# MDIL-SNU/SevenNet

Hardware: NVIDIA H100
Metric: atom_updates_per_sec (higher is better)
Workload: dtype f32

## Files before the change

sevenn_b200/csrc/engine.cu:

```cuda
#include <algorithm>
#include <cstdlib>
#include <cstring>
#include <functional>
#include <map>
#include <string>
#include <vector>

#include "../../include/sevenn_b200.h"
#include "common.cuh"
#include "conv_kernels.cuh"
#include "edge_kernels.cuh"
#include "neighbor.cuh"
#include "node_kernels.cuh"
#include "tc_gemm.cuh"

namespace s7b {

static thread_local std::string g_error;
static int64_t g_launches = 0;
extern int64_t g_conv_launches;

void set_error(const char* file, int line, const char* msg) {
  char buf[512];
  snprintf(buf, sizeof(buf), "%s:%d: %s", file, line, msg);
// ... 273 lines not shown
static int g_opt_gate_bwd_rows = 0;
static int g_opt_stage_graphs = 0;
static int g_opt_cuda_graph = 1;
static int g_opt_tc_gemm = 1;
static long long* g_tc_trace = nullptr;
static int g_tc_trace_cap = 0;
static int g_opt_tc_swizzle = 1;

__global__ void set_i64_kernel(int64_t* p, int64_t v) { *p = v; }

__global__ void csr_from_sorted_kernel(const int* __restrict__ centre, const int* __restrict__ neighbour,
                                       int64_t n_edges, int n_nodes, int* __restrict__ rowptr,
                                       int* __restrict__ flag) {
  const int64_t e = (int64_t)blockIdx.x * blockDim.x + threadIdx.x;
  if (e > n_edges) return;
  const int prev = (e == 0) ? -1 : centre[e - 1];
  const int cur = (e == n_edges) ? n_nodes : centre[e];
  if (e < n_edges) {
    if (cur < prev || cur < 0 || cur >= n_nodes) { atomicOr(flag, 1); return; }
    const int nb = neighbour[e];
    if (nb < 0 || nb >= n_nodes) atomicOr(flag, 2);
  }
  for (int c = max(prev, -1) + 1; c <= min(cur, n_nodes); ++c) rowptr[c] = (int)e;
}

__global__ void transpose_kernel(const float* __restrict__ in, float* __restrict__ out, int K, int N) {
  const size_t total = (size_t)K * N;
  for (size_t i = (size_t)blockIdx.x * blockDim.x + threadIdx.x; i < total; i += (size_t)gridDim.x * blockDim.x) {
    const int n = (int)(i / K), k = (int)(i - (size_t)n * K);
    out[i] = in[(size_t)k * N + n];
  }
}

struct TcWeights {
  DevBuf q, fb;
  int nblocks = 0;
  bool ok = false;
  struct Blk { int K, N, NT; size_t q_off, fb_off; } blk[kMaxL];
};

static int tc_pick_nt(int N) {
  if (N <= 0) return 0;
  const int tiles = (N + kTcMaxNT - 1) / kTcMaxNT;
  const int w = (N + tiles - 1) / tiles;
  return (w + 15) / 16 * 16;
}
static int tc_tiles(int N, int NT) { return (N + NT - 1) / NT; }

static inline uint16_t bf16_bits_exact(float v) {
  uint32_t u;
  memcpy(&u, &v, 4);
  return (uint16_t)(u >> 16);
}

static void tc_pack_block(const float* W, int K, int N, int NT, uint16_t* q, float* fb) {
  const int n_kc = K / kTcKC;
  for (int n = 0; n < N; ++n) {
    double amax = 0.0;
    for (int k = 0; k < K; ++k) amax = std::max(amax, (double)fabsf(W[(size_t)k * N + n]));
    int Eb = 0;
    const bool zero = !(amax > 1e-30);
    if (!zero) frexp(amax, &Eb);
    fb[n] = zero ? 0.0f : (float)ldexp(1.0, Eb - 7);
    const int nt = n / NT, r = n % NT;
    for (int k = 0; k < K; ++k) {
      double sl[3] = {0.0, 0.0, 0.0};
      if (!zero) {
        const double t = ldexp((double)W[(size_t)k * N + n], 23 - Eb);
        const double q0 = nearbyint(t / 65536.0);
        const double r1 = t - q0 * 65536.0;
        const double q1 = nearbyint(r1 / 256.0);
        const double r2 = r1 - q1 * 256.0;
        const double q2 = nearbyint(r2);
        sl[0] = q0; sl[1] = q1 / 256.0; sl[2] = q2 / 65536.0;
      }
      const int kc = k / kTcKC, kk = k % kTcKC;
      const size_t elem = (size_t)((r & 7) * 16 + (r >> 3) * 512 + (kk >> 3) * 128 + (kk & 7) * 2) / 2;
      for (int sidx = 0; sidx < 3; ++sidx)
        q[(((size_t)nt * n_kc + kc) * 3 + sidx) * ((size_t)NT * kTcKC) + elem] = bf16_bits_exact((float)sl[sidx]);
    }
  }
}

static int tc_build_weights(TcWeights& w, const float* host, const int* Ks, const int* Ns, int n_l) {
  w.ok = false;
  w.nblocks = 0;
  size_t q_total = 0, fb_total = 0, woff = 0;
  for (int l = 0; l < n_l; ++l) {
    const int K = Ks[l], N = Ns[l];
    if (K == 0 || N == 0) continue;
    const int NT = tc_pick_nt(N);
    if (NT == 0 || K % kTcKC != 0) return 0;
    TcWeights::Blk& b = w.blk[w.nblocks++];
    b = {K, N, NT, q_total, fb_total};
    q_total += (size_t)3 * K * NT * tc_tiles(N, NT);
    fb_total += (size_t)N;
  }
  std::vector<uint16_t> q(q_total);
  std::vector<float> fb(fb_total);
  int bi = 0;
  for (int l = 0; l < n_l; ++l) {
    const int K = Ks[l], N = Ns[l];
    if (K == 0 || N == 0) continue;
    const TcWeights::Blk& b = w.blk[bi++];
    tc_pack_block(host + woff, K, N, b.NT, q.data() + b.q_off, fb.data() + b.fb_off);
    woff += (size_t)K * N;
  }
  if (w.q.ensure(q_total * sizeof(uint16_t) + 16) || w.fb.ensure(fb_total * sizeof(float) + 16)) return fail("cudaMalloc failed for tensor-core weights");
  S7B_CUDA_CHECK(cudaMemcpy(w.q.p, q.data(), q_total * sizeof(uint16_t), cudaMemcpyHostToDevice));
  S7B_CUDA_CHECK(cudaMemcpy(w.fb.p, fb.data(), fb_total * sizeof(float), cudaMemcpyHostToDevice));
  w.ok = true;
  return 0;
}

typedef CUresult (*EncodeTiledFn)(CUtensorMap*, CUtensorMapDataType, cuuint32_t, void*, const cuuint64_t*, const cuuint64_t*,
                                  const cuuint32_t*, const cuuint32_t*, CUtensorMapInterleave, CUtensorMapSwizzle,
                                  CUtensorMapL2promotion, CUtensorMapFloatOOBfill);
static EncodeTiledFn tensor_map_encoder() {
  static EncodeTiledFn fn = nullptr;
  if (!fn) {
    void* p = nullptr;
    cudaDriverEntryPointQueryResult q;
    if (cudaGetDriverEntryPoint("cuTensorMapEncodeTiled", &p, cudaEnableDefault, &q) == cudaSuccess && q == cudaDriverEntryPointSuccess)
      fn = reinterpret_cast<EncodeTiledFn>(p);
    else cudaGetLastError();
  }
  return fn;
}

static int launch_row_exponents(RowExp& re, const float* A, int lda, const int* a_off, const int* a_K, int n_l,
                                int n_nodes, cudaStream_t st) {
  RowExpArgs r;
  memset(&r, 0, sizeof(r));
  r.A = A;
  r.lda = lda;
  r.n_nodes = n_nodes;
  int rows = 0;
  for (int l = 0; l < n_l; ++l) {
    if (a_K[l] == 0) continue;
    if (a_K[l] % 4 != 0) return fail("row exponents need K % 4 == 0");
    const int b = r.nblocks++;
    r.d[b] = 2 * l + 1;
    r.K[b] = a_K[l];
    r.a_off[b] = a_off[l];
    r.row_base[b] = rows;
    rows += 2 * l + 1;
  }
  r.rows_per_node = rows;
  re.rows_per_node = rows;
  re.bits = false;
  if (rows == 0 || n_nodes == 0) return 0;
  if (re.buf.ensure((size_t)n_nodes * rows * sizeof(int))) return fail("cudaMalloc failed for row exponents");
  r.E = re.buf.as<int>();
  if (rows > 16) return fail("row exponents: more than 16 rows per node");
  const int blk = 256, wpb = blk / 32;
  row_exponent_kernel<<<(n_nodes + wpb - 1) / wpb, blk, 0, st>>>(r);
  S7B_LAUNCH_CHECK();
  return 0;
}

static int launch_tc_linear(const TcWeights& w, const RowExp& re, const float* A, int lda, const int* a_off,
                            const int* a_K, float* C, int ldc, const int* c_off, const int* c_N, int n_l,
                            int n_nodes, bool accumulate, cudaStream_t st) {
  EncodeTiledFn enc = tensor_map_encoder();
  if (!enc) return fail("cuTensorMapEncodeTiled is unavailable (driver too old?)");
  if (ldc % 4 != 0 || (reinterpret_cast<uintptr_t>(C) & 15) != 0) return fail("tensor-core linear: C rows must be 16-byte aligned");
  for (int l = 0; l < n_l; ++l)
    if (c_N[l] != 0 && a_K[l] != 0 && (c_N[l] % 4 != 0 || c_off[l] % 4 != 0)) return fail("tensor-core linear: output blocks must be multiples of 4 floats");
  TcLinArgs t;
  TcMaps maps;
  memset(&t, 0, sizeof(t));
  memset(&maps, 0, sizeof(maps));
  t.C = C;
  t.E = re.buf.as<int>();
  t.ldc = ldc;
  t.n_nodes = n_nodes;
  t.rows_per_node = re.rows_per_node;
  t.accumulate = accumulate ? 1 : 0;
  t.swizzle = g_opt_tc_swizzle;
  t.e_bits = re.bits ? 1 : 0;
  t.trace = g_tc_trace;
  t.trace_cap = g_tc_trace_cap;
  const int n_mt = (n_nodes + kTcBM - 1) / kTcBM;
  int tiles = 0, rows = 0, bi = 0;
  for (int l = 0; l < n_l; ++l) {
    if (a_K[l] == 0 || c_N[l] == 0) { if (a_K[l] != 0) rows += 2 * l + 1; continue; }
    if (bi >= w.nblocks || w.blk[bi].K != a_K[l] || w.blk[bi].N != c_N[l]) return fail("tensor-core weights do not match the call");
    TcLinBlock& b = t.blk[t.nblocks];
// ... 1339 lines not shown
```

sevenn_b200/csrc/tc_gemm.cuh:

```cuda
#pragma once
#include <cuda.h>
#include <cuda_bf16.h>

#include <type_traits>

#include "common.cuh"
#include "node_kernels.cuh"

namespace s7b {

constexpr int kTcBM = 64;
constexpr int kTcKC = 32;
constexpr int kTcMaxNT = 128;
constexpr int kTcAccRegs = kTcMaxNT / 2;
constexpr int kTcThreads = 320;
constexpr int kTcXformThreads = 128;
constexpr int kTcMmaWarps = 4;
constexpr int kTcRawBytes = kTcBM * kTcKC * 4;
constexpr int kTcASliceBytes = kTcBM * kTcKC * 2;
constexpr int kTcBSliceBytes = kTcMaxNT * kTcKC * 2;
constexpr int kTcRawStages = 4, kTcOpsStages = 3, kTcWStages = 5;
constexpr int kTcOpsBytes = 3 * kTcASliceBytes, kTcWBytes = 3 * kTcBSliceBytes;
constexpr int kTcCBox = 16;
constexpr int kTcCBoxBytes = kTcBM * kTcCBox * 4;
constexpr int kTcCBytes = kTcBM * kTcMaxNT * 4;
constexpr int kTcRawOff = 0;
constexpr int kTcOpsOff = kTcRawOff + kTcRawStages * kTcRawBytes;
constexpr int kTcWOff = kTcOpsOff + kTcOpsStages * kTcOpsBytes;
constexpr int kTcCOff = kTcWOff + kTcWStages * kTcWBytes;
constexpr int kTcSmemBytes = kTcCOff + kTcCBytes + 1024 ;
static_assert(kTcCOff % 1024 == 0, "the swizzled C staging tile must be 1024-byte aligned");
constexpr int kTcZeroRow = -1000;

__device__ __forceinline__ uint32_t smem_u32(const void* p) {
  return static_cast<uint32_t>(__cvta_generic_to_shared(p));
}
__device__ __forceinline__ void mbar_init(uint64_t* bar, uint32_t count) {
  asm volatile("mbarrier.init.shared::cta.b64 [%0], %1;" ::"r"(smem_u32(bar)), "r"(count) : "memory");
}
__device__ __forceinline__ void mbar_wait(uint64_t* bar, uint32_t parity) {
  asm volatile(
      "{\n"
      ".reg .pred P1;\n"
      "LAB_WAIT:\n"
      "mbarrier.try_wait.parity.shared::cta.b64 P1, [%0], %1;\n"
      "@P1 bra DONE;\n"
      "bra LAB_WAIT;\n"
      "DONE:\n"
      "}\n" ::"r"(smem_u32(bar)), "r"(parity) : "memory");
}
__device__ __forceinline__ void mbar_arrive(uint64_t* bar) {
  asm volatile("mbarrier.arrive.shared::cta.b64 _, [%0];" ::"r"(smem_u32(bar)) : "memory");
}
__device__ __forceinline__ void mbar_arrive_after(uint64_t* bar, float dep) {
  asm volatile(
      "{\n"
      ".reg .pred p;\n"
      "setp.ne.b32 p, %1, 0x7fc12345;\n"
      "@p mbarrier.arrive.shared::cta.b64 _, [%0];\n"
      "}\n" ::"r"(smem_u32(bar)), "r"(__float_as_uint(dep)) : "memory");
}
__device__ __forceinline__ void mbar_expect_tx(uint64_t* bar, uint32_t bytes) {
  asm volatile("mbarrier.arrive.expect_tx.shared::cta.b64 _, [%0], %1;" ::"r"(smem_u32(bar)), "r"(bytes) : "memory");
}
__device__ __forceinline__ void fence_async_smem() { asm volatile("fence.proxy.async.shared::cta;" ::: "memory"); }

__device__ __forceinline__ void tma_load_3d(void* dst, const CUtensorMap* map, int c0, int c1, int c2, uint64_t* bar) {
  asm volatile(
      "cp.async.bulk.tensor.3d.shared::cluster.global.tile.mbarrier::complete_tx::bytes [%0], [%1, {%2, %3, %4}], [%5];"
      ::"r"(smem_u32(dst)), "l"(reinterpret_cast<uint64_t>(map)), "r"(c0), "r"(c1), "r"(c2), "r"(smem_u32(bar))
      : "memory");
}
__device__ __forceinline__ void bulk_load(void* dst, const void* src, uint32_t bytes, uint64_t* bar) {
  asm volatile(
      "cp.async.bulk.shared::cluster.global.mbarrier::complete_tx::bytes [%0], [%1], %2, [%3];"
      ::"r"(smem_u32(dst)), "l"(reinterpret_cast<uint64_t>(src)), "r"(bytes), "r"(smem_u32(bar))
      : "memory");
}
__device__ __forceinline__ void tma_store_3d(const CUtensorMap* map, uint32_t src, int c0, int c1, int c2) {
  asm volatile("cp.async.bulk.tensor.3d.global.shared::cta.tile.bulk_group [%0, {%1, %2, %3}], [%4];"
               ::"l"(reinterpret_cast<uint64_t>(map)), "r"(c0), "r"(c1), "r"(c2), "r"(src) : "memory");
}
__device__ __forceinline__ void tma_reduce_add_3d(const CUtensorMap* map, uint32_t src, int c0, int c1, int c2) {
  asm volatile("cp.reduce.async.bulk.tensor.3d.global.shared::cta.add.tile.bulk_group [%0, {%1, %2, %3}], [%4];"
               ::"l"(reinterpret_cast<uint64_t>(map)), "r"(c0), "r"(c1), "r"(c2), "r"(src) : "memory");
}
__device__ __forceinline__ void bulk_commit() { asm volatile("cp.async.bulk.commit_group;" ::: "memory"); }
__device__ __forceinline__ void bulk_wait_read_all() { asm volatile("cp.async.bulk.wait_group.read 0;" ::: "memory"); }
__device__ __forceinline__ void bulk_wait_all() { asm volatile("cp.async.bulk.wait_group 0;" ::: "memory"); }
__device__ __forceinline__ void mma_group_sync() { asm volatile("bar.sync 1, 128;" ::: "memory"); }
__device__ __forceinline__ void sts64(uint32_t saddr, float x, float y) {
  asm volatile("st.shared.v2.f32 [%0], {%1, %2};" ::"r"(saddr), "f"(x), "f"(y) : "memory");
}

__device__ __forceinline__ uint64_t gmma_desc(uint32_t saddr) {
  return (uint64_t)((saddr & 0x3FFFF) >> 4) | ((uint64_t)(128 >> 4) << 16) | ((uint64_t)(512 >> 4) << 32);
}
__device__ __forceinline__ void wgmma_fence() { asm volatile("wgmma.fence.sync.aligned;" ::: "memory"); }
__device__ __forceinline__ void wgmma_commit() { asm volatile("wgmma.commit_group.sync.aligned;" ::: "memory"); }
template <int N>
__device__ __forceinline__ void wgmma_wait() { asm volatile("wgmma.wait_group.sync.aligned %0;" ::"n"(N) : "memory"); }
__device__ __forceinline__ void acc_fence(float (&d)[kTcAccRegs]) {
#pragma unroll
  for (int i = 0; i < kTcAccRegs; ++i) asm volatile("" : "+f"(d[i])::"memory");
}
template <int N>
__device__ __forceinline__ void wgmma_bf16(float (&d)[kTcAccRegs], uint64_t da, uint64_t db, uint32_t scale_d);
template <> __device__ __forceinline__ void wgmma_bf16<16>(float (&d)[kTcAccRegs], uint64_t da, uint64_t db, uint32_t scale_d) {
  asm volatile(
      "{\n.reg .pred p;\nsetp.ne.b32 p, %10, 0;\n"
      "wgmma.mma_async.sync.aligned.m64n16k16.f32.bf16.bf16 {%0, %1, %2, %3, %4, %5, %6, %7}, %8, %9, p, 1, 1, 0, 0;\n}\n"
      : "+f"(d[0]), "+f"(d[1]), "+f"(d[2]), "+f"(d[3]), "+f"(d[4]), "+f"(d[5]), "+f"(d[6]), "+f"(d[7])
      : "l"(da), "l"(db), "r"(scale_d));
}
template <> __device__ __forceinline__ void wgmma_bf16<32>(float (&d)[kTcAccRegs], uint64_t da, uint64_t db, uint32_t scale_d) {
  asm volatile(
      "{\n.reg .pred p;\nsetp.ne.b32 p, %18, 0;\n"
      "wgmma.mma_async.sync.aligned.m64n32k16.f32.bf16.bf16 {%0, %1, %2, %3, %4, %5, %6, %7, %8, %9, %10, %11, %12, %13, %14, %15}, %16, %17, p, 1, 1, 0, 0;\n}\n"
      : "+f"(d[0]), "+f"(d[1]), "+f"(d[2]), "+f"(d[3]), "+f"(d[4]), "+f"(d[5]), "+f"(d[6]), "+f"(d[7]), "+f"(d[8]), "+f"(d[9]), "+f"(d[10]), "+f"(d[11]), "+f"(d[12]), "+f"(d[13]), "+f"(d[14]), "+f"(d[15])
      : "l"(da), "l"(db), "r"(scale_d));
}
template <> __device__ __forceinline__ void wgmma_bf16<48>(float (&d)[kTcAccRegs], uint64_t da, uint64_t db, uint32_t scale_d) {
  asm volatile(
      "{\n.reg .pred p;\nsetp.ne.b32 p, %26, 0;\n"
      "wgmma.mma_async.sync.aligned.m64n48k16.f32.bf16.bf16 {%0, %1, %2, %3, %4, %5, %6, %7, %8, %9, %10, %11, %12, %13, %14, %15, %16, %17, %18, %19, %20, %21, %22, %23}, %24, %25, p, 1, 1, 0, 0;\n}\n"
      : "+f"(d[0]), "+f"(d[1]), "+f"(d[2]), "+f"(d[3]), "+f"(d[4]), "+f"(d[5]), "+f"(d[6]), "+f"(d[7]), "+f"(d[8]), "+f"(d[9]), "+f"(d[10]), "+f"(d[11]), "+f"(d[12]), "+f"(d[13]), "+f"(d[14]), "+f"(d[15]), "+f"(d[16]), "+f"(d[17]), "+f"(d[18]), "+f"(d[19]), "+f"(d[20]), "+f"(d[21]), "+f"(d[22]), "+f"(d[23])
      : "l"(da), "l"(db), "r"(scale_d));
}
template <> __device__ __forceinline__ void wgmma_bf16<64>(float (&d)[kTcAccRegs], uint64_t da, uint64_t db, uint32_t scale_d) {
  asm volatile(
      "{\n.reg .pred p;\nsetp.ne.b32 p, %34, 0;\n"
      "wgmma.mma_async.sync.aligned.m64n64k16.f32.bf16.bf16 {%0, %1, %2, %3, %4, %5, %6, %7, %8, %9, %10, %11, %12, %13, %14, %15, %16, %17, %18, %19, %20, %21, %22, %23, %24, %25, %26, %27, %28, %29, %30, %31}, %32, %33, p, 1, 1, 0, 0;\n}\n"
      : "+f"(d[0]), "+f"(d[1]), "+f"(d[2]), "+f"(d[3]), "+f"(d[4]), "+f"(d[5]), "+f"(d[6]), "+f"(d[7]), "+f"(d[8]), "+f"(d[9]), "+f"(d[10]), "+f"(d[11]), "+f"(d[12]), "+f"(d[13]), "+f"(d[14]), "+f"(d[15]), "+f"(d[16]), "+f"(d[17]), "+f"(d[18]), "+f"(d[19]), "+f"(d[20]), "+f"(d[21]), "+f"(d[22]), "+f"(d[23]), "+f"(d[24]), "+f"(d[25]), "+f"(d[26]), "+f"(d[27]), "+f"(d[28]), "+f"(d[29]), "+f"(d[30]), "+f"(d[31])
      : "l"(da), "l"(db), "r"(scale_d));
}
template <> __device__ __forceinline__ void wgmma_bf16<80>(float (&d)[kTcAccRegs], uint64_t da, uint64_t db, uint32_t scale_d) {
  asm volatile(
      "{\n.reg .pred p;\nsetp.ne.b32 p, %42, 0;\n"
      "wgmma.mma_async.sync.aligned.m64n80k16.f32.bf16.bf16 {%0, %1, %2, %3, %4, %5, %6, %7, %8, %9, %10, %11, %12, %13, %14, %15, %16, %17, %18, %19, %20, %21, %22, %23, %24, %25, %26, %27, %28, %29, %30, %31, %32, %33, %34, %35, %36, %37, %38, %39}, %40, %41, p, 1, 1, 0, 0;\n}\n"
      : "+f"(d[0]), "+f"(d[1]), "+f"(d[2]), "+f"(d[3]), "+f"(d[4]), "+f"(d[5]), "+f"(d[6]), "+f"(d[7]), "+f"(d[8]), "+f"(d[9]), "+f"(d[10]), "+f"(d[11]), "+f"(d[12]), "+f"(d[13]), "+f"(d[14]), "+f"(d[15]), "+f"(d[16]), "+f"(d[17]), "+f"(d[18]), "+f"(d[19]), "+f"(d[20]), "+f"(d[21]), "+f"(d[22]), "+f"(d[23]), "+f"(d[24]), "+f"(d[25]), "+f"(d[26]), "+f"(d[27]), "+f"(d[28]), "+f"(d[29]), "+f"(d[30]), "+f"(d[31]), "+f"(d[32]), "+f"(d[33]), "+f"(d[34]), "+f"(d[35]), "+f"(d[36]), "+f"(d[37]), "+f"(d[38]), "+f"(d[39])
      : "l"(da), "l"(db), "r"(scale_d));
}
template <> __device__ __forceinline__ void wgmma_bf16<96>(float (&d)[kTcAccRegs], uint64_t da, uint64_t db, uint32_t scale_d) {
  asm volatile(
      "{\n.reg .pred p;\nsetp.ne.b32 p, %50, 0;\n"
      "wgmma.mma_async.sync.aligned.m64n96k16.f32.bf16.bf16 {%0, %1, %2, %3, %4, %5, %6, %7, %8, %9, %10, %11, %12, %13, %14, %15, %16, %17, %18, %19, %20, %21, %22, %23, %24, %25, %26, %27, %28, %29, %30, %31, %32, %33, %34, %35, %36, %37, %38, %39, %40, %41, %42, %43, %44, %45, %46, %47}, %48, %49, p, 1, 1, 0, 0;\n}\n"
      : "+f"(d[0]), "+f"(d[1]), "+f"(d[2]), "+f"(d[3]), "+f"(d[4]), "+f"(d[5]), "+f"(d[6]), "+f"(d[7]), "+f"(d[8]), "+f"(d[9]), "+f"(d[10]), "+f"(d[11]), "+f"(d[12]), "+f"(d[13]), "+f"(d[14]), "+f"(d[15]), "+f"(d[16]), "+f"(d[17]), "+f"(d[18]), "+f"(d[19]), "+f"(d[20]), "+f"(d[21]), "+f"(d[22]), "+f"(d[23]), "+f"(d[24]), "+f"(d[25]), "+f"(d[26]), "+f"(d[27]), "+f"(d[28]), "+f"(d[29]), "+f"(d[30]), "+f"(d[31]), "+f"(d[32]), "+f"(d[33]), "+f"(d[34]), "+f"(d[35]), "+f"(d[36]), "+f"(d[37]), "+f"(d[38]), "+f"(d[39]), "+f"(d[40]), "+f"(d[41]), "+f"(d[42]), "+f"(d[43]), "+f"(d[44]), "+f"(d[45]), "+f"(d[46]), "+f"(d[47])
      : "l"(da), "l"(db), "r"(scale_d));
}
template <> __device__ __forceinline__ void wgmma_bf16<112>(float (&d)[kTcAccRegs], uint64_t da, uint64_t db, uint32_t scale_d) {
  asm volatile(
      "{\n.reg .pred p;\nsetp.ne.b32 p, %58, 0;\n"
      "wgmma.mma_async.sync.aligned.m64n112k16.f32.bf16.bf16 {%0, %1, %2, %3, %4, %5, %6, %7, %8, %9, %10, %11, %12, %13, %14, %15, %16, %17, %18, %19, %20, %21, %22, %23, %24, %25, %26, %27, %28, %29, %30, %31, %32, %33, %34, %35, %36, %37, %38, %39, %40, %41, %42, %43, %44, %45, %46, %47, %48, %49, %50, %51, %52, %53, %54, %55}, %56, %57, p, 1, 1, 0, 0;\n}\n"
      : "+f"(d[0]), "+f"(d[1]), "+f"(d[2]), "+f"(d[3]), "+f"(d[4]), "+f"(d[5]), "+f"(d[6]), "+f"(d[7]), "+f"(d[8]), "+f"(d[9]), "+f"(d[10]), "+f"(d[11]), "+f"(d[12]), "+f"(d[13]), "+f"(d[14]), "+f"(d[15]), "+f"(d[16]), "+f"(d[17]), "+f"(d[18]), "+f"(d[19]), "+f"(d[20]), "+f"(d[21]), "+f"(d[22]), "+f"(d[23]), "+f"(d[24]), "+f"(d[25]), "+f"(d[26]), "+f"(d[27]), "+f"(d[28]), "+f"(d[29]), "+f"(d[30]), "+f"(d[31]), "+f"(d[32]), "+f"(d[33]), "+f"(d[34]), "+f"(d[35]), "+f"(d[36]), "+f"(d[37]), "+f"(d[38]), "+f"(d[39]), "+f"(d[40]), "+f"(d[41]), "+f"(d[42]), "+f"(d[43]), "+f"(d[44]), "+f"(d[45]), "+f"(d[46]), "+f"(d[47]), "+f"(d[48]), "+f"(d[49]), "+f"(d[50]), "+f"(d[51]), "+f"(d[52]), "+f"(d[53]), "+f"(d[54]), "+f"(d[55])
      : "l"(da), "l"(db), "r"(scale_d));
}
template <> __device__ __forceinline__ void wgmma_bf16<128>(float (&d)[kTcAccRegs], uint64_t da, uint64_t db, uint32_t scale_d) {
  asm volatile(
      "{\n.reg .pred p;\nsetp.ne.b32 p, %66, 0;\n"
      "wgmma.mma_async.sync.aligned.m64n128k16.f32.bf16.bf16 {%0, %1, %2, %3, %4, %5, %6, %7, %8, %9, %10, %11, %12, %13, %14, %15, %16, %17, %18, %19, %20, %21, %22, %23, %24, %25, %26, %27, %28, %29, %30, %31, %32, %33, %34, %35, %36, %37, %38, %39, %40, %41, %42, %43, %44, %45, %46, %47, %48, %49, %50, %51, %52, %53, %54, %55, %56, %57, %58, %59, %60, %61, %62, %63}, %64, %65, p, 1, 1, 0, 0;\n}\n"
      : "+f"(d[0]), "+f"(d[1]), "+f"(d[2]), "+f"(d[3]), "+f"(d[4]), "+f"(d[5]), "+f"(d[6]), "+f"(d[7]), "+f"(d[8]), "+f"(d[9]), "+f"(d[10]), "+f"(d[11]), "+f"(d[12]), "+f"(d[13]), "+f"(d[14]), "+f"(d[15]), "+f"(d[16]), "+f"(d[17]), "+f"(d[18]), "+f"(d[19]), "+f"(d[20]), "+f"(d[21]), "+f"(d[22]), "+f"(d[23]), "+f"(d[24]), "+f"(d[25]), "+f"(d[26]), "+f"(d[27]), "+f"(d[28]), "+f"(d[29]), "+f"(d[30]), "+f"(d[31]), "+f"(d[32]), "+f"(d[33]), "+f"(d[34]), "+f"(d[35]), "+f"(d[36]), "+f"(d[37]), "+f"(d[38]), "+f"(d[39]), "+f"(d[40]), "+f"(d[41]), "+f"(d[42]), "+f"(d[43]), "+f"(d[44]), "+f"(d[45]), "+f"(d[46]), "+f"(d[47]), "+f"(d[48]), "+f"(d[49]), "+f"(d[50]), "+f"(d[51]), "+f"(d[52]), "+f"(d[53]), "+f"(d[54]), "+f"(d[55]), "+f"(d[56]), "+f"(d[57]), "+f"(d[58]), "+f"(d[59]), "+f"(d[60]), "+f"(d[61]), "+f"(d[62]), "+f"(d[63])
      : "l"(da), "l"(db), "r"(scale_d));
}

__device__ __forceinline__ float exp2i(int e) {
  e = e < -126 ? -126 : (e > 127 ? 127 : e);
  return __int_as_float((e + 127) << 23);
}

struct RowExpArgs {
  const float* A;
  int* E;
  int lda, n_nodes, rows_per_node, nblocks;
  int d[kMaxL], K[kMaxL], a_off[kMaxL], row_base[kMaxL];
};

__global__ void row_exponent_kernel(const RowExpArgs a) {
  __shared__ unsigned int smax[8][16];
  const int wib = threadIdx.x >> 5, lane = threadIdx.x & 31;
  const int n = blockIdx.x * (blockDim.x >> 5) + wib;
  if (lane < 16) smax[wib][lane] = 0u;
  __syncwarp();
  if (n < a.n_nodes) {
    for (int b = 0; b < a.nblocks; ++b) {
      const int K = a.K[b], quads = (a.d[b] * K) >> 2;
      const float4* row = reinterpret_cast<const float4*>(a.A + (size_t)n * a.lda + a.a_off[b]);
      for (int q0 = 0; q0 < quads; q0 += 32) {
        const int q = q0 + lane;
        unsigned int m = 0u;
        int r = -1;
        if (q < quads) {
          const float4 v = __ldg(row + q);
          m = __float_as_uint(v.x) & 0x7fffffffu;
          m = max(m, __float_as_uint(v.y) & 0x7fffffffu);
          m = max(m, __float_as_uint(v.z) & 0x7fffffffu);
          m = max(m, __float_as_uint(v.w) & 0x7fffffffu);
          r = a.row_base[b] + (4 * q) / K;
        }
        const unsigned int peers = __match_any_sync(0xffffffffu, r);
        const unsigned int mm = __reduce_max_sync(peers, m);
        if (r >= 0 && lane == __ffs(peers) - 1) smax[wib][r] = max(smax[wib][r], mm);
        __syncwarp();
      }
    }
  }
  __syncwarp();
  if (n < a.n_nodes && lane < a.rows_per_node) {
    const int ex = (int)(smax[wib][lane] >> 23);
    a.E[(size_t)n * a.rows_per_node + lane] = (ex == 0 || ex == 255) ? kTcZeroRow : max(ex - 126, -104);
  }
}

struct TcLinBlock {
  const uint16_t* Wq;
  const float* fb;
  int d, K, N, NT, nnt;
  int c_off, c_cs;
  int row_base;
  int tile0;
};
struct TcLinArgs {
  float* C;
  const int* E;
  int ldc, n_nodes, rows_per_node, accumulate, nblocks, n_tiles, swizzle;
  int e_bits;
  long long* trace;
  int trace_cap;
  TcLinBlock blk[kMaxL];
};
#define TC_TRACE(role, ev, idx)                                                                   \
  do {                                                                                            \
    if (a.trace != nullptr && blockIdx.x == 0) {                                                  \
      const int per = a.trace_cap / 5;                                                            \
      if (trace_n < per) {                                                                        \
        long long* rec = a.trace + 8 + 3 * ((size_t)(role) * per + trace_n);                      \
        rec[0] = (ev);                                                                            \
        rec[1] = (long long)(idx);                                                                \
        rec[2] = clock64();                                                                       \
        ++trace_n;                                                                                \
        a.trace[1 + (role)] = trace_n;                                                            \
      }                                                                                           \
    }                                                                                             \
  } while (0)
struct TcMaps { CUtensorMap m[kMaxL], c[kMaxL]; };

__device__ __forceinline__ float4 lds128(uint32_t saddr) {
  float4 v;
  asm volatile("ld.shared.v4.f32 {%0, %1, %2, %3}, [%4];" : "=f"(v.x), "=f"(v.y), "=f"(v.z), "=f"(v.w) : "r"(saddr) : "memory");
  return v;
}
__device__ __forceinline__ void sts128(uint32_t saddr, uint32_t a, uint32_t b, uint32_t c, uint32_t d) {
  asm volatile("st.shared.v4.b32 [%0], {%1, %2, %3, %4};" ::"r"(saddr), "r"(a), "r"(b), "r"(c), "r"(d) : "memory");
}

__device__ __forceinline__ uint32_t pack_bf16(float lo, float hi) {
  const __nv_bfloat162 v = __floats2bfloat162_rn(lo, hi);
  return *reinterpret_cast<const uint32_t*>(&v);
}

template <int N>
__device__ __forceinline__ void tc_mma_chunk(float (&acc0)[kTcAccRegs], float (&acc1)[kTcAccRegs], uint32_t sa,
                                             uint32_t sb, bool first) {
  constexpr uint32_t b_slice = (uint32_t)N * kTcKC * 2u;
#pragma unroll
  for (int j = 0; j < kTcKC / 16; ++j) {
    const uint32_t ko = (uint32_t)j * 256u;
    const uint64_t dA0 = gmma_desc(sa + ko);
    const uint64_t dA1 = gmma_desc(sa + kTcASliceBytes + ko);
    const uint64_t dA2 = gmma_desc(sa + 2 * kTcASliceBytes + ko);
    const uint64_t dB0 = gmma_desc(sb + ko);
    const uint64_t dB1 = gmma_desc(sb + b_slice + ko);
    const uint64_t dB2 = gmma_desc(sb + 2 * b_slice + ko);
    const uint32_t acc = (!first || j > 0) ? 1u : 0u;
    wgmma_bf16<N>(acc0, dA0, dB0, acc);
    wgmma_bf16<N>(acc1, dA0, dB1, acc);
    wgmma_bf16<N>(acc1, dA1, dB0, 1u);
    wgmma_bf16<N>(acc1, dA0, dB2, 1u);
    wgmma_bf16<N>(acc1, dA1, dB1, 1u);
    wgmma_bf16<N>(acc1, dA2, dB0, 1u);
  }
}

__global__ void __launch_bounds__(kTcThreads, 1)
blocklin_tc_kernel(const TcLinArgs a, const __grid_constant__ TcMaps maps) {
  extern __shared__ uint8_t smem_raw[];
  uint8_t* smem = reinterpret_cast<uint8_t*>((reinterpret_cast<uintptr_t>(smem_raw) + 1023) & ~(uintptr_t)1023);
  __shared__ uint64_t bar_raw_full[kTcRawStages], bar_raw_empty[kTcRawStages];
  __shared__ uint64_t bar_ops_full[kTcOpsStages], bar_ops_empty[kTcOpsStages];
  __shared__ uint64_t bar_w_full[kTcWStages], bar_w_empty[kTcWStages];
  __shared__ __align__(16) float fb_s[kTcMaxNT];

  const int tid = threadIdx.x, warp = tid >> 5, lane = tid & 31;
  int trace_n = 0;

  if (tid == 0) {
    for (int s = 0; s < kTcRawStages; ++s) { mbar_init(&bar_raw_full[s], 1); mbar_init(&bar_raw_empty[s], kTcXformThreads); }
    for (int s = 0; s < kTcOpsStages; ++s) { mbar_init(&bar_ops_full[s], kTcXformThreads); mbar_init(&bar_ops_empty[s], kTcMmaWarps); }
    for (int s = 0; s < kTcWStages; ++s) { mbar_init(&bar_w_full[s], 1); mbar_init(&bar_w_empty[s], kTcMmaWarps); }
    asm volatile("fence.mbarrier_init.release.cluster;" ::: "memory");
  }
  __syncthreads();

  auto decode = [&](int t, int& b, int& mt, int& ci, int& nt) {
    b = 0;
    while (b + 1 < a.nblocks && t >= a.blk[b + 1].tile0) ++b;
    const int rel = t - a.blk[b].tile0;
    const int nnt = a.blk[b].nnt;
    nt = rel % nnt;
    const int r2 = rel / nnt;
    ci = r2 % a.blk[b].d;
    mt = r2 / a.blk[b].d;
  };
  auto row_exp = [&](int t, int row) -> int {
    if (t >= a.n_tiles) return kTcZeroRow;
    int b, mt, ci, nt;
    decode(t, b, mt, ci, nt);
    const int node = mt * kTcBM + row;
    if (node >= a.n_nodes) return kTcZeroRow;
    int v = __ldg(a.E + (size_t)node * a.rows_per_node + a.blk[b].row_base + ci);
    if (a.e_bits) {
      const int ex = v >> 23;
      v = (ex == 0 || ex == 255) ? kTcZeroRow : max(ex - 126, -104);
    }
    return v;
  };

  if (warp == 8) {
    if (lane == 0) {
      uint32_t it = 0;
      for (int t = blockIdx.x; t < a.n_tiles; t += gridDim.x) {
        int b, mt, ci, nt;
        decode(t, b, mt, ci, nt);
        const int n_kc = a.blk[b].K / kTcKC;
        for (int kc = 0; kc < n_kc; ++kc, ++it) {
          const int s = it % kTcRawStages;
          mbar_wait(&bar_raw_empty[s], ((it / kTcRawStages) & 1) ^ 1);
          TC_TRACE(0, 0, it);
          mbar_expect_tx(&bar_raw_full[s], (uint32_t)kTcRawBytes);
          tma_load_3d(smem + kTcRawOff + (size_t)s * kTcRawBytes, &maps.m[b], kc * kTcKC, ci, mt * kTcBM, &bar_raw_full[s]);
        }
      }
    }
  } else if (warp == 9) {
    if (lane == 0) {
      uint32_t it = 0;
      for (int t = blockIdx.x; t < a.n_tiles; t += gridDim.x) {
        int b, mt, ci, nt;
        decode(t, b, mt, ci, nt);
        const TcLinBlock& B = a.blk[b];
        const int n_kc = B.K / kTcKC;
        const uint32_t b_bytes = 3u * (uint32_t)B.NT * kTcKC * 2u;
        const uint8_t* wsrc = reinterpret_cast<const uint8_t*>(B.Wq) + (size_t)nt * n_kc * b_bytes;
        for (int kc = 0; kc < n_kc; ++kc, ++it) {
          const int s = it % kTcWStages;
          mbar_wait(&bar_w_empty[s], ((it / kTcWStages) & 1) ^ 1);
          TC_TRACE(4, 0, it);
          mbar_expect_tx(&bar_w_full[s], b_bytes);
          bulk_load(smem + kTcWOff + (size_t)s * kTcWBytes, wsrc + (size_t)kc * b_bytes, b_bytes, &bar_w_full[s]);
        }
      }
    }
  } else if (warp < 4) {
    const int r = tid & (kTcBM - 1), h = tid / kTcBM;
    const uint32_t swz = a.swizzle ? (uint32_t)(r & 7) : 0u;
    const uint32_t row_off = (uint32_t)((r & 7) * 16 + (r >> 3) * 512);
    const V2 M2 = splat2(12582912.0f), nM2 = splat2(-12582912.0f);
    uint32_t it = 0;
    int Ea_next = row_exp(blockIdx.x, r);
    for (int t = blockIdx.x; t < a.n_tiles; t += gridDim.x) {
      int b, mt, ci, nt;
      decode(t, b, mt, ci, nt);
      const int n_kc = a.blk[b].K / kTcKC;
      const int Ea = Ea_next;
      Ea_next = row_exp(t + gridDim.x, r);
      const float sc = (Ea == kTcZeroRow) ? 0.0f : exp2i(23 - Ea);
      for (int kc = 0; kc < n_kc; ++kc, ++it) {
        const int s = it % kTcRawStages, o = it % kTcOpsStages;
        mbar_wait(&bar_raw_full[s], (it / kTcRawStages) & 1);
        if (tid == 0) TC_TRACE(1, 0, it);
        const uint32_t raw = smem_u32(smem + kTcRawOff + (size_t)s * kTcRawBytes + (size_t)r * 128);
        float4 v[4];
#pragma unroll
        for (int q = 0; q < 4; ++q) v[q] = lds128(raw + (((uint32_t)(4 * h + q) ^ swz) << 4));
        const float dep = (v[0].x + v[1].x) + (v[2].x + v[3].x);
        mbar_arrive_after(&bar_raw_empty[s], dep);
        mbar_wait(&bar_ops_empty[o], ((it / kTcOpsStages) & 1) ^ 1);
        if (tid == 0) TC_TRACE(1, 1, it);
        const uint32_t a0 = smem_u32(smem + kTcOpsOff + (size_t)o * kTcOpsBytes);
        const uint32_t a1 = a0 + kTcASliceBytes, a2 = a1 + kTcASliceBytes;
#pragma unroll
        for (int kk = 0; kk < 2; ++kk) {
          const V2 x[4] = {make_float2(v[2 * kk].x, v[2 * kk].y), make_float2(v[2 * kk].z, v[2 * kk].w),
                           make_float2(v[2 * kk + 1].x, v[2 * kk + 1].y), make_float2(v[2 * kk + 1].z, v[2 * kk + 1].w)};
          uint32_t p0[4], p1[4], p2[4];
#pragma unroll
          for (int j = 0; j < 4; ++j) {
            const V2 tt = mul_(x[j], sc);
            const V2 q0 = add_(fma_(tt, splat2(1.52587890625e-05f), M2), nM2);
            const V2 r1 = fma_(q0, splat2(-65536.0f), tt);
            const V2 q1 = add_(fma_(r1, splat2(0.00390625f), M2), nM2);
            const V2 r2 = fma_(q1, splat2(-256.0f), r1);
            const V2 q2 = add_(add_(r2, M2), nM2);
            const V2 s1 = mul_(q1, 0.00390625f), s2 = mul_(q2, 1.52587890625e-05f);
            p0[j] = pack_bf16(q0.x, q0.y);
            p1[j] = pack_bf16(s1.x, s1.y);
            p2[j] = pack_bf16(s2.x, s2.y);
          }
          const uint32_t off = row_off + (uint32_t)(2 * h + kk) * 128u;
          sts128(a0 + off, p0[0], p0[1], p0[2], p0[3]);
          sts128(a1 + off, p1[0], p1[1], p1[2], p1[3]);
          sts128(a2 + off, p2[0], p2[1], p2[2], p2[3]);
        }
        fence_async_smem();
        if (tid == 0) TC_TRACE(1, 2, it);
        mbar_arrive(&bar_ops_full[o]);
      }
    }
  } else if (warp < 8) {
    const int mw = warp - 4, q4 = lane & 3, ct = tid - 128;
    const int rl = 16 * mw + (lane >> 2);
    const uint32_t cst = smem_u32(smem + kTcCOff);
    auto c_addr = [&](int r, int j) -> uint32_t {
      const int g = 2 * (j & 1) + (q4 >> 1);
      return cst + (uint32_t)((j >> 1) * kTcCBoxBytes + r * 64 + ((g ^ ((r >> 1) & 3)) << 4) + (q4 & 1) * 8);
    };
    float acc0[kTcAccRegs], acc1[kTcAccRegs];
#pragma unroll
    for (int i = 0; i < kTcAccRegs; ++i) { acc0[i] = 0.0f; acc1[i] = 0.0f; }
    uint32_t it = 0, tile_it = 0;
    int Ea_next0 = row_exp(blockIdx.x, rl), Ea_next1 = row_exp(blockIdx.x, rl + 8);
    for (int t = blockIdx.x; t < a.n_tiles; t += gridDim.x, ++tile_it) {
      int b, mt, ci, nt;
      decode(t, b, mt, ci, nt);
      const TcLinBlock& B = a.blk[b];
      const int n_kc = B.K / kTcKC;
      const int Ea0 = Ea_next0, Ea1 = Ea_next1;
      Ea_next0 = row_exp(t + gridDim.x, rl);
      Ea_next1 = row_exp(t + gridDim.x, rl + 8);
      const int col0 = nt * B.NT;
      const float fb_t = (ct < B.NT && col0 + ct < B.N) ? __ldg(B.fb + col0 + ct) : 0.0f;
      auto run_tile = [&](auto width) {
        constexpr int N = decltype(width)::value;
        int prev_o = 0, prev_w = 0;
        for (int kc = 0; kc < n_kc; ++kc, ++it) {
          const int o = it % kTcOpsStages, w = it % kTcWStages;
          mbar_wait(&bar_w_full[w], (it / kTcWStages) & 1);
          if (tid == 128) TC_TRACE(2, 0, it);
          mbar_wait(&bar_ops_full[o], (it / kTcOpsStages) & 1);
          if (tid == 128) TC_TRACE(2, 1, it);
          __syncwarp();
          const uint32_t sa = smem_u32(smem + kTcOpsOff + (size_t)o * kTcOpsBytes);
          const uint32_t sb = smem_u32(smem + kTcWOff + (size_t)w * kTcWBytes);
          acc_fence(acc0);
          acc_fence(acc1);
          wgmma_fence();
          tc_mma_chunk<N>(acc0, acc1, sa, sb, kc == 0);
          wgmma_commit();
          acc_fence(acc0);
          acc_fence(acc1);
          wgmma_wait<1>();
          if (kc > 0) {
            __syncwarp();
            if (lane == 0) { mbar_arrive(&bar_ops_empty[prev_o]); mbar_arrive(&bar_w_empty[prev_w]); }
          }
          prev_o = o;
          prev_w = w;
        }
        wgmma_wait<0>();
        acc_fence(acc0);
        acc_fence(acc1);
        __syncwarp();
        if (lane == 0) { mbar_arrive(&bar_ops_empty[prev_o]); mbar_arrive(&bar_w_empty[prev_w]); }
        if (tid == 160) TC_TRACE(3, 0, tile_it);

        const float fa0 = (Ea0 == kTcZeroRow) ? 0.0f : exp2i(Ea0 - 7);
        const float fa1 = (Ea1 == kTcZeroRow) ? 0.0f : exp2i(Ea1 - 7);
        if (tid == 128) bulk_wait_read_all();
        fb_s[ct] = fb_t;
        mma_group_sync();
        if (tid == 160) TC_TRACE(3, 2, tile_it);
#pragma unroll
        for (int j = 0; j < N / 8; ++j) {
          const float2 fb2 = *reinterpret_cast<const float2*>(&fb_s[8 * j + 2 * q4]);
          sts64(c_addr(rl, j), (acc0[4 * j + 0] + acc1[4 * j + 0]) * fa0 * fb2.x,
                (acc0[4 * j + 1] + acc1[4 * j + 1]) * fa0 * fb2.y);
          sts64(c_addr(rl + 8, j), (acc0[4 * j + 2] + acc1[4 * j + 2]) * fa1 * fb2.x,
                (acc0[4 * j + 3] + acc1[4 * j + 3]) * fa1 * fb2.y);
        }
        if (tid == 160) TC_TRACE(3, 3, tile_it);
      };
      switch (B.NT) {
        case 16: run_tile(std::integral_constant<int, 16>()); break;
        case 32: run_tile(std::integral_constant<int, 32>()); break;
        case 48: run_tile(std::integral_constant<int, 48>()); break;
        case 64: run_tile(std::integral_constant<int, 64>()); break;
        case 80: run_tile(std::integral_constant<int, 80>()); break;
        case 96: run_tile(std::integral_constant<int, 96>()); break;
        case 112: run_tile(std::integral_constant<int, 112>()); break;
        default: run_tile(std::integral_constant<int, 128>()); break;
      }
      fence_async_smem();
      mma_group_sync();
      if (tid == 128) {
        for (int s = 0; s < B.NT / kTcCBox && col0 + s * kTcCBox < B.N; ++s) {
          const uint32_t src = cst + (uint32_t)(s * kTcCBoxBytes);
          if (a.accumulate) tma_reduce_add_3d(&maps.c[b], src, col0 + s * kTcCBox, ci, mt * kTcBM);
          else tma_store_3d(&maps.c[b], src, col0 + s * kTcCBox, ci, mt * kTcBM);
        }
        bulk_commit();
      }
      if (tid == 160) TC_TRACE(3, 1, tile_it);
    }
    if (tid == 128) bulk_wait_all();
  }
}

}
```

Baseline: 1.414 million.

## Ping-pong two MMA warpgroups with dedicated store warp and 64B swizzled operands

Adds a second consumer warpgroup so two MMA groups alternate tiles, each running its epilogue while the other runs tensor-core MMAs. A dedicated warp now issues the TMA stores and reduce-adds for the C staging tile. setmaxnreg rebalances registers toward the MMA warps. Weights and transformed A operands are also switched to a 64-byte swizzled shared-memory layout to cut bank conflicts. The cost is more threads and more mbarrier coordination. The single C staging buffer is still shared between the groups, so their epilogues serialize on it.

```diff
diff --git a/sevenn_b200/csrc/engine.cu b/sevenn_b200/csrc/engine.cu
--- a/sevenn_b200/csrc/engine.cu
+++ b/sevenn_b200/csrc/engine.cu
@@ -379,6 +379,17 @@
   }
 }
 
+static void tc_swizzle_block(uint16_t* q, size_t elems, int NT) {
+  const size_t piece = (size_t)NT * kTcKC;
+  std::vector<uint16_t> tmp(piece);
+  for (size_t p0 = 0; p0 < elems; p0 += piece) {
+    for (int r = 0; r < NT; ++r)
+      for (int g = 0; g < kTcKC / 8; ++g)
+        memcpy(tmp.data() + tc_swz64((uint32_t)r, (uint32_t)g) / 2, q + p0 + ((r & 7) * 16 + (r >> 3) * 512 + g * 128) / 2, 16);
+    memcpy(q + p0, tmp.data(), piece * sizeof(uint16_t));
+  }
+}
+
 static int tc_build_weights(TcWeights& w, const float* host, const int* Ks, const int* Ns, int n_l) {
   w.ok = false;
   w.nblocks = 0;
@@ -401,6 +412,7 @@
     if (K == 0 || N == 0) continue;
     const TcWeights::Blk& b = w.blk[bi++];
     tc_pack_block(host + woff, K, N, b.NT, q.data() + b.q_off, fb.data() + b.fb_off);
+    tc_swizzle_block(q.data() + b.q_off, (size_t)3 * K * b.NT * tc_tiles(N, b.NT), b.NT);
     woff += (size_t)K * N;
   }
   if (w.q.ensure(q_total * sizeof(uint16_t) + 16) || w.fb.ensure(fb_total * sizeof(float) + 16)) return fail("cudaMalloc failed for tensor-core weights");
diff --git a/sevenn_b200/csrc/tc_gemm.cuh b/sevenn_b200/csrc/tc_gemm.cuh
--- a/sevenn_b200/csrc/tc_gemm.cuh
+++ b/sevenn_b200/csrc/tc_gemm.cuh
@@ -13,7 +13,8 @@
 constexpr int kTcKC = 32;
 constexpr int kTcMaxNT = 128;
 constexpr int kTcAccRegs = kTcMaxNT / 2;
-constexpr int kTcThreads = 320;
+constexpr int kTcThreads = 512;
+constexpr int kTcXformRegs = 88, kTcProdRegs = 40, kTcMmaRegs = 192;
 constexpr int kTcXformThreads = 128;
 constexpr int kTcMmaWarps = 4;
 constexpr int kTcRawBytes = kTcBM * kTcKC * 4;
@@ -88,14 +89,17 @@
 __device__ __forceinline__ void bulk_commit() { asm volatile("cp.async.bulk.commit_group;" ::: "memory"); }
 __device__ __forceinline__ void bulk_wait_read_all() { asm volatile("cp.async.bulk.wait_group.read 0;" ::: "memory"); }
 __device__ __forceinline__ void bulk_wait_all() { asm volatile("cp.async.bulk.wait_group 0;" ::: "memory"); }
-__device__ __forceinline__ void mma_group_sync() { asm volatile("bar.sync 1, 128;" ::: "memory"); }
+__device__ __forceinline__ void mma_group_sync(int g) { asm volatile("bar.sync %0, 128;" ::"r"(1 + g) : "memory"); }
+template <int R> __device__ __forceinline__ void setmaxnreg_inc() { asm volatile("setmaxnreg.inc.sync.aligned.u32 %0;" ::"n"(R)); }
+template <int R> __device__ __forceinline__ void setmaxnreg_dec() { asm volatile("setmaxnreg.dec.sync.aligned.u32 %0;" ::"n"(R)); }
 __device__ __forceinline__ void sts64(uint32_t saddr, float x, float y) {
   asm volatile("st.shared.v2.f32 [%0], {%1, %2};" ::"r"(saddr), "f"(x), "f"(y) : "memory");
 }
 
 __device__ __forceinline__ uint64_t gmma_desc(uint32_t saddr) {
-  return (uint64_t)((saddr & 0x3FFFF) >> 4) | ((uint64_t)(128 >> 4) << 16) | ((uint64_t)(512 >> 4) << 32);
-}
+  return (uint64_t)((saddr & 0x3FFFF) >> 4) | ((uint64_t)1 << 16) | ((uint64_t)(512 >> 4) << 32) | ((uint64_t)2 << 62);
+}
+__host__ __device__ __forceinline__ uint32_t tc_swz64(uint32_t r, uint32_t g) { return r * 64u + ((g ^ ((r >> 1) & 3u)) << 4); }
 __device__ __forceinline__ void wgmma_fence() { asm volatile("wgmma.fence.sync.aligned;" ::: "memory"); }
 __device__ __forceinline__ void wgmma_commit() { asm volatile("wgmma.commit_group.sync.aligned;" ::: "memory"); }
 template <int N>
@@ -231,7 +235,7 @@
 #define TC_TRACE(role, ev, idx)                                                                   \
   do {                                                                                            \
     if (a.trace != nullptr && blockIdx.x == 0) {                                                  \
-      const int per = a.trace_cap / 5;                                                            \
+      const int per = a.trace_cap / 7;                                                            \
       if (trace_n < per) {                                                                        \
         long long* rec = a.trace + 8 + 3 * ((size_t)(role) * per + trace_n);                      \
         rec[0] = (ev);                                                                            \
@@ -264,7 +268,7 @@
   constexpr uint32_t b_slice = (uint32_t)N * kTcKC * 2u;
 #pragma unroll
   for (int j = 0; j < kTcKC / 16; ++j) {
-    const uint32_t ko = (uint32_t)j * 256u;
+    const uint32_t ko = (uint32_t)j * 32u;
     const uint64_t dA0 = gmma_desc(sa + ko);
     const uint64_t dA1 = gmma_desc(sa + kTcASliceBytes + ko);
     const uint64_t dA2 = gmma_desc(sa + 2 * kTcASliceBytes + ko);
@@ -288,7 +292,9 @@
   __shared__ uint64_t bar_raw_full[kTcRawStages], bar_raw_empty[kTcRawStages];
   __shared__ uint64_t bar_ops_full[kTcOpsStages], bar_ops_empty[kTcOpsStages];
   __shared__ uint64_t bar_w_full[kTcWStages], bar_w_empty[kTcWStages];
-  __shared__ __align__(16) float fb_s[kTcMaxNT];
+  __shared__ uint64_t bar_c_full, bar_c_free[2];
+  __shared__ uint64_t bar_turn[2];
+  __shared__ __align__(16) float fb_s[2][kTcMaxNT];
 
   const int tid = threadIdx.x, warp = tid >> 5, lane = tid & 31;
   int trace_n = 0;
@@ -297,6 +303,11 @@
     for (int s = 0; s < kTcRawStages; ++s) { mbar_init(&bar_raw_full[s], 1); mbar_init(&bar_raw_empty[s], kTcXformThreads); }
     for (int s = 0; s < kTcOpsStages; ++s) { mbar_init(&bar_ops_full[s], kTcXformThreads); mbar_init(&bar_ops_empty[s], kTcMmaWarps); }
     for (int s = 0; s < kTcWStages; ++s) { mbar_init(&bar_w_full[s], 1); mbar_init(&bar_w_empty[s], kTcMmaWarps); }
+    mbar_init(&bar_c_full, 1);
+    mbar_init(&bar_c_free[0], 1);
+    mbar_init(&bar_c_free[1], 1);
+    mbar_init(&bar_turn[0], kTcMmaWarps);
+    mbar_init(&bar_turn[1], kTcMmaWarps);
     asm volatile("fence.mbarrier_init.release.cluster;" ::: "memory");
   }
   __syncthreads();
@@ -325,8 +336,9 @@
     return v;
   };
 
-  if (warp == 8) {
-    if (lane == 0) {
+  if (warp >= 4 && warp < 8) {
+    setmaxnreg_dec<kTcProdRegs>();
+    if (warp == 4 && lane == 0) {
       uint32_t it = 0;
       for (int t = blockIdx.x; t < a.n_tiles; t += gridDim.x) {
         int b, mt, ci, nt;
@@ -340,9 +352,7 @@
           tma_load_3d(smem + kTcRawOff + (size_t)s * kTcRawBytes, &maps.m[b], kc * kTcKC, ci, mt * kTcBM, &bar_raw_full[s]);
         }
       }
-    }
-  } else if (warp == 9) {
-    if (lane == 0) {
+    } else if (warp == 5 && lane == 0) {
       uint32_t it = 0;
       for (int t = blockIdx.x; t < a.n_tiles; t += gridDim.x) {
         int b, mt, ci, nt;
@@ -359,11 +369,30 @@
           bulk_load(smem + kTcWOff + (size_t)s * kTcWBytes, wsrc + (size_t)kc * b_bytes, b_bytes, &bar_w_full[s]);
         }
       }
+    } else if (warp == 6 && lane == 0) {
+      uint32_t s = 0;
+      for (int t = blockIdx.x; t < a.n_tiles; t += gridDim.x, ++s) {
+        int b, mt, ci, nt;
+        decode(t, b, mt, ci, nt);
+        const TcLinBlock& B = a.blk[b];
+        const int col0 = nt * B.NT;
+        mbar_wait(&bar_c_full, s & 1);
+        const uint32_t cst = smem_u32(smem + kTcCOff);
+        for (int q = 0; q < B.NT / kTcCBox && col0 + q * kTcCBox < B.N; ++q) {
+          const uint32_t src = cst + (uint32_t)(q * kTcCBoxBytes);
+          if (a.accumulate) tma_reduce_add_3d(&maps.c[b], src, col0 + q * kTcCBox, ci, mt * kTcBM);
+          else tma_store_3d(&maps.c[b], src, col0 + q * kTcCBox, ci, mt * kTcBM);
+        }
+        bulk_commit();
+        bulk_wait_read_all();
+        mbar_arrive(&bar_c_free[(s + 1) & 1]);
+      }
+      bulk_wait_all();
     }
   } else if (warp < 4) {
+    setmaxnreg_dec<kTcXformRegs>();
     const int r = tid & (kTcBM - 1), h = tid / kTcBM;
     const uint32_t swz = a.swizzle ? (uint32_t)(r & 7) : 0u;
-    const uint32_t row_off = (uint32_t)((r & 7) * 16 + (r >> 3) * 512);
     const V2 M2 = splat2(12582912.0f), nM2 = splat2(-12582912.0f);
     uint32_t it = 0;
     int Ea_next = row_exp(blockIdx.x, r);
@@ -406,7 +435,7 @@
             p1[j] = pack_bf16(s1.x, s1.y);
             p2[j] = pack_bf16(s2.x, s2.y);
           }
-          const uint32_t off = row_off + (uint32_t)(2 * h + kk) * 128u;
+          const uint32_t off = tc_swz64((uint32_t)r, (uint32_t)(2 * h + kk));
           sts128(a0 + off, p0[0], p0[1], p0[2], p0[3]);
           sts128(a1 + off, p1[0], p1[1], p1[2], p1[3]);
           sts128(a2 + off, p2[0], p2[1], p2[2], p2[3]);
@@ -416,27 +445,29 @@
         mbar_arrive(&bar_ops_full[o]);
       }
     }
-  } else if (warp < 8) {
-    const int mw = warp - 4, q4 = lane & 3, ct = tid - 128;
+  } else {
+    setmaxnreg_inc<kTcMmaRegs>();
+    const int g = (warp - 8) >> 2, mw = (warp - 8) & 3, q4 = lane & 3, ct = tid & 127;
     const int rl = 16 * mw + (lane >> 2);
+    const bool tr_mma = (ct == 0), tr_epi = (ct == 32);
+    const int role_mma = g ? 5 : 2, role_epi = g ? 6 : 3;
     const uint32_t cst = smem_u32(smem + kTcCOff);
+    float* fbs = fb_s[g];
     auto c_addr = [&](int r, int j) -> uint32_t {
-      const int g = 2 * (j & 1) + (q4 >> 1);
-      return cst + (uint32_t)((j >> 1) * kTcCBoxBytes + r * 64 + ((g ^ ((r >> 1) & 3)) << 4) + (q4 & 1) * 8);
+      const int gr = 2 * (j & 1) + (q4 >> 1);
+      return cst + (uint32_t)((j >> 1) * kTcCBoxBytes + r * 64 + ((gr ^ ((r >> 1) & 3)) << 4) + (q4 & 1) * 8);
     };
     float acc0[kTcAccRegs], acc1[kTcAccRegs];
 #pragma unroll
     for (int i = 0; i < kTcAccRegs; ++i) { acc0[i] = 0.0f; acc1[i] = 0.0f; }
-    uint32_t it = 0, tile_it = 0;
-    int Ea_next0 = row_exp(blockIdx.x, rl), Ea_next1 = row_exp(blockIdx.x, rl + 8);
+    uint32_t it = 0, tile_it = 0, mine = 0;
     for (int t = blockIdx.x; t < a.n_tiles; t += gridDim.x, ++tile_it) {
       int b, mt, ci, nt;
       decode(t, b, mt, ci, nt);
       const TcLinBlock& B = a.blk[b];
       const int n_kc = B.K / kTcKC;
-      const int Ea0 = Ea_next0, Ea1 = Ea_next1;
-      Ea_next0 = row_exp(t + gridDim.x, rl);
-      Ea_next1 = row_exp(t + gridDim.x, rl + 8);
+      if ((int)(tile_it & 1) != g) { it += n_kc; continue; }
+      const int Ea0 = row_exp(t, rl), Ea1 = row_exp(t, rl + 8);
       const int col0 = nt * B.NT;
       const float fb_t = (ct < B.NT && col0 + ct < B.N) ? __ldg(B.fb + col0 + ct) : 0.0f;
       auto run_tile = [&](auto width) {
@@ -445,9 +476,9 @@
         for (int kc = 0; kc < n_kc; ++kc, ++it) {
           const int o = it % kTcOpsStages, w = it % kTcWStages;
           mbar_wait(&bar_w_full[w], (it / kTcWStages) & 1);
-          if (tid == 128) TC_TRACE(2, 0, it);
+          if (tr_mma) TC_TRACE(role_mma, 0, it);
           mbar_wait(&bar_ops_full[o], (it / kTcOpsStages) & 1);
-          if (tid == 128) TC_TRACE(2, 1, it);
+          if (tr_mma) TC_TRACE(role_mma, 1, it);
           __syncwarp();
           const uint32_t sa = smem_u32(smem + kTcOpsOff + (size_t)o * kTcOpsBytes);
           const uint32_t sb = smem_u32(smem + kTcWOff + (size_t)w * kTcWBytes);
@@ -459,6 +490,7 @@
           acc_fence(acc0);
           acc_fence(acc1);
           wgmma_wait<1>();
+          if (tr_mma) TC_TRACE(role_mma, 2, it);
           if (kc > 0) {
             __syncwarp();
             if (lane == 0) { mbar_arrive(&bar_ops_empty[prev_o]); mbar_arrive(&bar_w_empty[prev_w]); }
@@ -466,29 +498,32 @@
           prev_o = o;
           prev_w = w;
         }
+        __syncwarp();
+        if (lane == 0) mbar_arrive(&bar_turn[g ^ 1]);
         wgmma_wait<0>();
         acc_fence(acc0);
         acc_fence(acc1);
         __syncwarp();
         if (lane == 0) { mbar_arrive(&bar_ops_empty[prev_o]); mbar_arrive(&bar_w_empty[prev_w]); }
-        if (tid == 160) TC_TRACE(3, 0, tile_it);
+        if (tr_epi) TC_TRACE(role_epi, 0, tile_it);
 
         const float fa0 = (Ea0 == kTcZeroRow) ? 0.0f : exp2i(Ea0 - 7);
         const float fa1 = (Ea1 == kTcZeroRow) ? 0.0f : exp2i(Ea1 - 7);
-        if (tid == 128) bulk_wait_read_all();
-        fb_s[ct] = fb_t;
-        mma_group_sync();
-        if (tid == 160) TC_TRACE(3, 2, tile_it);
+        fbs[ct] = fb_t;
+        mbar_wait(&bar_c_free[g], (mine & 1) ^ (uint32_t)(g ^ 1));
+        mma_group_sync(g);
+        if (tr_epi) TC_TRACE(role_epi, 2, tile_it);
 #pragma unroll
         for (int j = 0; j < N / 8; ++j) {
-          const float2 fb2 = *reinterpret_cast<const float2*>(&fb_s[8 * j + 2 * q4]);
+          const float2 fb2 = *reinterpret_cast<const float2*>(&fbs[8 * j + 2 * q4]);
           sts64(c_addr(rl, j), (acc0[4 * j + 0] + acc1[4 * j + 0]) * fa0 * fb2.x,
                 (acc0[4 * j + 1] + acc1[4 * j + 1]) * fa0 * fb2.y);
           sts64(c_addr(rl + 8, j), (acc0[4 * j + 2] + acc1[4 * j + 2]) * fa1 * fb2.x,
                 (acc0[4 * j + 3] + acc1[4 * j + 3]) * fa1 * fb2.y);
         }
-        if (tid == 160) TC_TRACE(3, 3, tile_it);
+        if (tr_epi) TC_TRACE(role_epi, 3, tile_it);
       };
+      mbar_wait(&bar_turn[g], (mine & 1) ^ (uint32_t)(g ^ 1));
       switch (B.NT) {
         case 16: run_tile(std::integral_constant<int, 16>()); break;
         case 32: run_tile(std::integral_constant<int, 32>()); break;
@@ -500,18 +535,11 @@
         default: run_tile(std::integral_constant<int, 128>()); break;
       }
       fence_async_smem();
-      mma_group_sync();
-      if (tid == 128) {
-        for (int s = 0; s < B.NT / kTcCBox && col0 + s * kTcCBox < B.N; ++s) {
-          const uint32_t src = cst + (uint32_t)(s * kTcCBoxBytes);
-          if (a.accumulate) tma_reduce_add_3d(&maps.c[b], src, col0 + s * kTcCBox, ci, mt * kTcBM);
-          else tma_store_3d(&maps.c[b], src, col0 + s * kTcCBox, ci, mt * kTcBM);
-        }
-        bulk_commit();
-      }
-      if (tid == 160) TC_TRACE(3, 1, tile_it);
+      mma_group_sync(g);
+      if (ct == 0) mbar_arrive(&bar_c_full);
+      if (tr_epi) TC_TRACE(role_epi, 1, tile_it);
+      ++mine;
     }
-    if (tid == 128) bulk_wait_all();
   }
 }
 
```

Result: faster. 1.489 million (median of 6 runs) (+5.3%).
